# andrewdalpino/UltraZoom

Hardware: AMD Instinct MI355X
Metric: upscaled MPix/sec, MewZoom-4X 1080p bf16 batched inference (higher is better)
Workload: dtype bf16; 1 GPU; MewZoom-4X 96ch/40L bf16, 16 x 1080x1920 -> 4320x7680 per GPU; global_batch=16, parallelism=batch-sharded x1, images_in_flight=0

## Files before the change

### include/mewzoom_hip.h

```cpp
#ifndef MEWZOOM_HIP_H
#define MEWZOOM_HIP_H

#include <stddef.h>
#include <stdint.h>

#ifdef __cplusplus
extern "C" {
#endif

typedef struct mz_handle mz_handle;

typedef enum mz_dtype {
    MZ_F32 = 0,
    MZ_BF16 = 1,
    MZ_F16 = 2
} mz_dtype;

typedef enum mz_status {
    MZ_OK = 0,
    MZ_ERR_INVALID_ARGUMENT = -1,
    MZ_ERR_UNKNOWN_WEIGHT = -2,
    MZ_ERR_SHAPE_MISMATCH = -3,
    MZ_ERR_MISSING_WEIGHTS = -4,
    MZ_ERR_WORKSPACE_TOO_SMALL = -5,
// ... 100 lines not shown
const char* mz_version(void);
double mz_flops_per_image(const mz_handle* h, int H, int W);
int mz_profile_enable(mz_handle* h, int on);
int mz_profile_dump(mz_handle* h, const char* path);
int mz_profile_read(mz_handle* h, double* conv_ms, double* conv_flops, double* conv_launches,
                    double* other_ms, double* conv_bytes);

int mz_debug_read(unsigned long long* host_dst);

const char* mz_debug_last_kernel(void);

int mz_debug_tile_list(int B, int tiles_y, int tiles_x, int ntiles, int gm, int gn, int blk4, int th, int tw, unsigned int* out, int cap);

const char* mz_debug_select(int dtype, int op, int cin, int cout, int B, int H, int W, int cus);

typedef struct mz_debug_step {
    int32_t kind, op, cin, cout, B, H, W, Hout, Wout, fused;
    int64_t off[3];
    uint64_t bytes[3];
    const char* kernel;
} mz_debug_step;

int mz_debug_schedule(const mz_handle* h, int B, int H, int W, int want_qa, int cus, mz_debug_step* out, int cap);

long long mz_debug_pack(int dtype, int op, int cin, int cout, int layout, long long* out, long long cap);

int mz_debug_store_hazard(int follower, int form, int wait_states, int dword, int iters, int blocks, unsigned int* counts_out);

#ifdef __cplusplus
}
// ... 3 lines not shown
```

### ultrazoom_amd/csrc/mz_conv3r.h

```cpp
#pragma once
#include "mz_device.h"
#include "mz_diag.h"
#include "mz_relay.h"

namespace mz {
namespace r3 {

constexpr int TH = 8;
template <int GEO> struct Geo {
    static_assert(GEO == 0 || GEO == 1, "8 x 48 or 8 x 40");
    static constexpr int TW = GEO == 0 ? 48 : 40;
    static constexpr int NPF = GEO == 0 ? 6 : 5;
    static constexpr int ROWW = TW + 2;
    static constexpr int NPIX = 10 * ROWW;
    static constexpr int DIV_MAGIC = GEO == 0 ? 1311 : 1561;
    static constexpr int X0 = 3, X1 = NPF - 3;
    static constexpr bool straddle(int pf) { return GEO == 1 && pf == 2; }
    static constexpr int dy(int pf) { return GEO == 0 ? pf / 3 : (pf >= 3 ? 1 : 0); }
    static constexpr int dx(int pf) { return GEO == 0 ? 16 * (pf % 3) : (pf < 2 ? 16 * pf : (pf == 2 ? 0 : 8 + 16 * (pf - 3))); }
};
constexpr int PLANE_ENT = 512;
constexpr int A_PLANE = PLANE_ENT * 16;
constexpr int A_SLOT = 4 * A_PLANE;
constexpr int NT = 3, NF = 6, BN = 96;
constexpr int NG = 9 * NT;
constexpr int B_BASE = 2 * A_SLOT;
constexpr int CHUNK_PIECES = 2 * NG;
constexpr int MIX_PIECES = 4 * NT * NT;

template <int NSEG> struct Seg {
    static_assert(NSEG == 2 || NSEG == 3, "two or three weight segments per chunk");
    static constexpr int start(int s) { return NSEG == 2 ? (s <= 0 ? 0 : (s == 1 ? (NG + 1) / 2 : NG)) : (NG / 3) * s; }
    static constexpr int of(int G) { return NSEG == 2 ? (G < start(1) ? 0 : 1) : G / (NG / 3); }
    static constexpr int pieces(int s) { return 2 * (start(s + 1) - start(s)); }
    static constexpr int SLOT = pieces(0) * 1024;
    static constexpr int MIX_BASE = B_BASE + 3 * SLOT;
    static constexpr int lds_bytes(bool fuse) { return fuse ? MIX_BASE + MIX_PIECES * 1024 : B_BASE + 3 * SLOT; }
};

template <int GEO, int TAP, int PF> constexpr int a_off() {
    using GG = Geo<GEO>;
    constexpr int DY = TAP / 3, DX = TAP % 3;
    return ((DY + GG::dy(PF)) * GG::ROWW + DX + GG::dx(PF)) * 16;
}

template <int NPF> struct Frag {
    u32x4 x[2][NPF];
    u32x4 w[3][2];
};

template <int N> __device__ __forceinline__ void wait_w(u32x4& w0, u32x4& w1) {
    asm volatile("s_waitcnt lgkmcnt(%2)" : "+v"(w0), "+v"(w1) : "n"(N) : "memory");
// ... 95 lines not shown
        gate_wait<(more ? NT : 0)>(wa);
        __builtin_amdgcn_sched_barrier(0);
#pragma unroll
        for (int i = 0; i < NT; ++i) {
            if constexpr (ks == 0) mma16_first<TT>(beta[part * NT + i], wa[i], xf[0]);
            else if constexpr (ks < NT) mma16<TT>(beta[part * NT + i], wa[i], xf[ks]);
            else mma16<TT>(beta[part * NT + i], wa[i], zf[ks - NT]);
        }
        __builtin_amdgcn_sched_barrier(0);
        gate_halves<TT, H + 1>(beta, xf, zf, wb, wa, addr);
    }
}

}

template <class TT, int NSEG, int EPI, bool SILU, int GEO = 0, bool RAG = false>
__global__ __launch_bounds__(512) void conv3r_kernel(const ConvArgs a) {
    using namespace r3;
    using namespace relay;
    using S = Seg<NSEG>;
    using GG = Geo<GEO>;
    constexpr int NPF = GG::NPF, TW = GG::TW, ROWW = GG::ROWW, NPIX = GG::NPIX;
    constexpr int NE = NPF * NT;
    constexpr bool FUSE = EPI == EPI_FUSEDMIX;
    static_assert(!FUSE || GEO == 0, "the fused variant is built for the 8 x 48 tile");
    constexpr int B_SLOT = S::SLOT;
    static_assert(!FUSE || NSEG == 3, "the gate weights need the LDS that three weight segments leave free");
    static_assert(!RAG || (NSEG == 3 && EPI == EPI_STORE && GEO == 0), "the ragged two-chunk variant: three steps per chunk, plain stores, 8 x 48 tiles");
    extern __shared__ __attribute__((aligned(16))) char smem[];
    const int w = __builtin_amdgcn_readfirstlane((int)threadIdx.x >> 6);
    const int team = w >> 2, wq = w & 3;
    const int nchunks = a.nchunks16;
    const uint32_t lds_base = (uint32_t)(uintptr_t)(__attribute__((address_space(3))) char*)smem;

    const int xcd = blockIdx.x & 7, pos = blockIdx.x >> 3, step = gridDim.x >> 3;
    const int q = a.grid >> 3, rem = a.grid & 7;
    const int cnt = q + (xcd < rem ? 1 : 0);
    const int base = xcd < rem ? xcd * (q + 1) : rem * (q + 1) + (xcd - rem) * q;
    if (pos >= cnt) return;
    typedef uint32_t TabE __attribute__((ext_vector_type(2)));
    typedef const __attribute__((address_space(4))) TabE* TabPtr;
    const TabPtr tab = (TabPtr)(uintptr_t)a.tile_tab + base;
    struct TileE { uint32_t yx, bn; };
// ... 217 lines not shown
    auto entry_whole = [&](auto e_tag) __attribute__((always_inline)) {
        if constexpr (decltype(e_tag)::value < NE) {
            u32x4 o;
            entry_words(e_tag, o);
            epi_store(e_tag, o);
        }
    };

    auto prime = [&](int wslot, int aslot) __attribute__((always_inline)) {
        const int lane_ = lane_now();
        const int g = lane_ >> 4, c = lane_ & 15;
        Bases pb;
        pb.a_cur = pb.a_nxt = lds_base + aslot * A_SLOT + g * A_PLANE + ((2 * wq) * ROWW + c) * 16;
        pb.a2_cur = pb.a2_nxt = pb.a_cur + (uint32_t)((c >= 8 ? ROWW - 8 : 32) * 16);
        pb.b_cur = pb.b_nxt = 0;
        const uint32_t bb = lds_base + B_BASE + wslot * B_SLOT + lane_ * 16;
        f.x[0][0] = read_x<GEO, 0, 0>(pb, false);
        f.x[0][1] = read_x<GEO, 0, 1>(pb, false);
        f.x[0][2] = read_x<GEO, 0, 2>(pb, false);
        f.x[0][3] = read_x<GEO, 0, 3>(pb, false);
        f.x[0][4] = read_x<GEO, 0, 4>(pb, false);
        if constexpr (NPF > 5) f.x[0][NPF - 1] = read_x<GEO, 0, NPF - 1>(pb, false);
        f.w[0][0] = lds_read128<0 * 1024>(bb);
        f.w[0][1] = lds_read128<1 * 1024>(bb);
        f.w[1][0] = lds_read128<2 * 1024>(bb);
        f.w[1][1] = lds_read128<3 * 1024>(bb);
        wait_wx<0>(f.w[0][0], f.w[0][1], f.x[0]);
        wait_w<0>(f.w[1][0], f.w[1][1]);
    };

    const char* wA = nullptr;
    const char* wB = nullptr;
    bool okB = false;
    auto loader_step = [&](auto wk_tag, auto es_tag, auto en_tag, auto sg_tag, auto last_tag, int k) __attribute__((always_inline)) {
        constexpr int WK = decltype(wk_tag)::value;
        constexpr int ES = decltype(es_tag)::value, EN = WK == 0 ? 0 : decltype(en_tag)::value, sg = decltype(sg_tag)::value;
        constexpr bool last = decltype(last_tag)::value != 0;
        [[maybe_unused]] constexpr int rs_c = 1 + (EN > 0 ? 2 : 0) + (sg == 0 ? 0 : 1);
        static_assert(EN <= 3, "three output registers");
        constexpr int VM_AFTER0 = WK == 1 ? EN : (WK == 2 ? (ES + 1 < NPF ? NF : 0) : (WK == 4 ? EN * NT : 0));
        constexpr int VM_AFTER = VM_AFTER0 + (NSEG == 3 && sg == 0 ? 8 : 0);
        RS_BEGIN();
        if constexpr (WK == 2 && ES == 0) fuse_x(ic<0>{});
        if constexpr (WK == 3) x_landed(ic<ES>{});
        constexpr bool HALO_LATE = NSEG == 3;
        auto halo_image = [&]() __attribute__((always_inline)) {
            const __amdgpu_buffer_rsrc_t h_rsrc = halo_rsrc(last ? 0 : k + 1);
            uint32_t h_off = (uint32_t)(us ^ 1) * (uint32_t)A_SLOT;
// ... 4 lines not shown
            halo_piece(ic<3>{}, h_rsrc, h_dst, rag); halo_piece(ic<4>{}, h_rsrc, h_dst, rag); halo_piece(ic<5>{}, h_rsrc, h_dst, rag);
            halo_piece(ic<6>{}, h_rsrc, h_dst, rag); halo_piece(ic<7>{}, h_rsrc, h_dst, rag);
        };
        if constexpr (sg == 0 && !HALO_LATE) {
            if (!last || okB) halo_image();
        }
        {
            constexpr bool same = sg + 2 < NSEG;
            constexpr int qs = same ? sg + 2 : sg + 2 - NSEG;
            const char* wsrc;
            bool w_ok = true;
            if constexpr (same) wsrc = wA + (size_t)k * chunk_bytes;
            else if constexpr (!last) wsrc = wA + (size_t)(k + 1) * chunk_bytes;
            else { wsrc = wB; w_ok = okB; }
            wsrc += (size_t)(2 * S::start(qs)) * 1024;
            const int w_pieces = w_ok ? wseg_count(S::pieces(qs)) : 0;
            char* const w_dst = smem + B_BASE + (hs >= 1 ? hs - 1 : 2) * B_SLOT;
            const uint32_t lo = (uint32_t)lane_now() * 16u;
            wseg_piece(ic<0>{}, wsrc, w_pieces, w_dst, lo); wseg_piece(ic<1>{}, wsrc, w_pieces, w_dst, lo); wseg_piece(ic<2>{}, wsrc, w_pieces, w_dst, lo);
            wseg_piece(ic<3>{}, wsrc, w_pieces, w_dst, lo); wseg_piece(ic<4>{}, wsrc, w_pieces, w_dst, lo);
            if constexpr (WP > 5) wseg_piece(ic<5>{}, wsrc, w_pieces, w_dst, lo);
            if constexpr (WP > 6) wseg_piece(ic<6>{}, wsrc, w_pieces, w_dst, lo);
            static_assert(WP <= 7, "seven weight pieces per wave and step");
        }
        if constexpr (sg == 0 && HALO_LATE) halo_image();
        __builtin_amdgcn_sched_barrier(0);
        asm volatile("" ::: "memory");
        RS_LAP(4 * rs_c);
        if constexpr (WK == 1) {
            u32x4 o0, o1, o2;
            if constexpr (EN > 0) entry_words(ic<ES>{}, o0);
            if constexpr (EN > 1) entry_words(ic<ES + 1>{}, o1);
// ... 48 lines not shown
    auto fuse_chunk = [&](auto p0_tag, auto g_tag, auto last_tag, int k) __attribute__((always_inline)) {
        static_assert(!FUSE || NSEG == 3, "the fused variant runs three steps per chunk");
        loader_step(ic<2>{}, p0_tag, g_tag, ic<0>{}, last_tag, k);
        loader_step(ic<3>{}, p0_tag, g_tag, ic<1>{}, last_tag, k);
        loader_step(ic<4>{}, p0_tag, g_tag, ic<NSEG - 1>{}, last_tag, k);
    };
    auto plain_chunks = [&](int k0) __attribute__((always_inline)) {
        for (int k = k0; k + 1 < nchunks; ++k) loader_chunk(ic<0>{}, ic<0>{}, ic<0>{}, ic<0>{}, k);
        loader_chunk(ic<0>{}, ic<0>{}, ic<0>{}, ic<1>{}, nchunks - 1);
    };
    auto loader_phase = [&](auto epi_tag) __attribute__((always_inline)) {
        constexpr bool DO_EPI = decltype(epi_tag)::value != 0;
        wA = wsrc_of(tile_nt(eA));
        okB = a_pos + step < cnt;
        wB = wsrc_of(tile_nt(okB ? eB : eA));
        const TileE eA2 = tile_at(a_pos + 2 * step), eB2 = tile_at(a_pos + 3 * step);
        if constexpr (DO_EPI) {
            RS_BEGIN();
            set_load_tile(eA);
            epi_setup();
            RS_FENCE();
            RS_LAP(27);
            if constexpr (RAG) {
                loader_chunk(ic<0>{}, ic<3>{}, ic<6>{}, ic<0>{}, 0);
                loader_chunk(ic<9>{}, ic<3>{}, ic<6>{}, ic<1>{}, 1);
            } else if constexpr (FUSE) {
                fuse_chunk(ic<0>{}, ic<1>{}, ic<0>{}, 0);
                fuse_chunk(ic<1>{}, ic<1>{}, ic<0>{}, 1);
                fuse_chunk(ic<2>{}, ic<1>{}, ic<0>{}, 2);
                fuse_chunk(ic<3>{}, ic<1>{}, ic<0>{}, 3);
// ... 33 lines not shown
        eD = eB; eA = eA2; eB = eB2;
        asm volatile("" ::"s"(eA.yx), "s"(eA.bn), "s"(eB.yx), "s"(eB.bn));
    };

    auto compute_phase = [&]() __attribute__((always_inline)) {
        const int lane_ = lane_now();
        const int g = lane_ >> 4, c = lane_ & 15;
        const uint32_t a_lane = lds_base + g * A_PLANE + ((2 * wq) * ROWW + c) * 16;
        Bases bs;
        bs.a_cur = a_lane + us * A_SLOT;
        bs.a_nxt = a_lane + (us ^ 1) * A_SLOT;
        const uint32_t a_str = (uint32_t)((c >= 8 ? ROWW - 8 : 32) * 16);
        bs.a2_cur = bs.a_cur + a_str;
        bs.a2_nxt = bs.a_nxt + a_str;
        const uint32_t bl = lds_base + B_BASE + lane_ * 16;
        uint32_t b0 = bl + hs * B_SLOT, b1 = bl + next3(hs) * B_SLOT, b2 = bl + next3(next3(hs)) * B_SLOT;
        bs.b_cur = b0;
        bs.b_nxt = b1;
        auto step_tail = [&]() __attribute__((always_inline)) {
            __builtin_amdgcn_s_barrier();
            const uint32_t u_ = b0; b0 = b1; b1 = b2; b2 = u_;
            bs.b_cur = b0; bs.b_nxt = b1;
        };
        auto chunk = [&](auto xp_tag, bool first) __attribute__((always_inline)) {
            constexpr int XP = decltype(xp_tag)::value;
            groups<TT, NSEG, GEO, S::start(0), S::start(1), XP>(acc, f, bs, first);
            step_tail();
            groups<TT, NSEG, GEO, S::start(1), S::start(2), XP>(acc, f, bs, false);
            step_tail();
            if constexpr (NSEG == 3) {
                groups<TT, NSEG, GEO, S::start(2), S::start(3), XP>(acc, f, bs, false);
                step_tail();
            }
            const uint32_t v_ = bs.a_cur; bs.a_cur = bs.a_nxt; bs.a_nxt = v_;
            if constexpr (GEO == 1) { const uint32_t v2_ = bs.a2_cur; bs.a2_cur = bs.a2_nxt; bs.a2_nxt = v2_; }
        };
        RS_BEGIN();
        int kc = 0;
        for (;;) {
            chunk(ic<0>{}, !FUSE && kc == 0);
            if (++kc >= nchunks) break;
            chunk(ic<1>{}, false);
            if (++kc >= nchunks) break;
        }
        asm volatile("s_waitcnt lgkmcnt(0)"
                     : "+v"(f.x[0][0]), "+v"(f.x[0][1]), "+v"(f.x[0][2]), "+v"(f.x[0][3]), "+v"(f.x[0][4]), "+v"(f.x[0][NPF - 1]),
                       "+v"(f.x[1][0]), "+v"(f.x[1][1]), "+v"(f.x[1][2]), "+v"(f.x[1][3]), "+v"(f.x[1][4]), "+v"(f.x[1][NPF - 1])
// ... 26 lines not shown
        }
    };

    if (team == 1) {
        eA = tile_at(a_pos);
        eB = tile_at(a_pos + step);
        eD = eA;
        wA = wsrc_of(tile_nt(eA));
        set_load_tile(eA);
        {
            const __amdgpu_buffer_rsrc_t r0 = halo_rsrc(0);
            halo_piece(ic<0>{}, r0, smem); halo_piece(ic<1>{}, r0, smem); halo_piece(ic<2>{}, r0, smem); halo_piece(ic<3>{}, r0, smem);
            halo_piece(ic<4>{}, r0, smem); halo_piece(ic<5>{}, r0, smem); halo_piece(ic<6>{}, r0, smem); halo_piece(ic<7>{}, r0, smem);
            const char* s1 = wA + (size_t)(2 * S::start(1)) * 1024;
            const uint32_t lo = (uint32_t)lane_now() * 16u;
            char* d0 = smem + B_BASE;
            char* d1 = smem + B_BASE + B_SLOT;
            wseg_piece(ic<0>{}, wA, wseg_count(S::pieces(0)), d0, lo); wseg_piece(ic<1>{}, wA, wseg_count(S::pieces(0)), d0, lo); wseg_piece(ic<2>{}, wA, wseg_count(S::pieces(0)), d0, lo);
            wseg_piece(ic<3>{}, wA, wseg_count(S::pieces(0)), d0, lo); wseg_piece(ic<4>{}, wA, wseg_count(S::pieces(0)), d0, lo); wseg_piece(ic<5>{}, wA, wseg_count(S::pieces(0)), d0, lo);
            wseg_piece(ic<6>{}, wA, wseg_count(S::pieces(0)), d0, lo);
            wseg_piece(ic<0>{}, s1, wseg_count(S::pieces(1)), d1, lo); wseg_piece(ic<1>{}, s1, wseg_count(S::pieces(1)), d1, lo); wseg_piece(ic<2>{}, s1, wseg_count(S::pieces(1)), d1, lo);
            wseg_piece(ic<3>{}, s1, wseg_count(S::pieces(1)), d1, lo); wseg_piece(ic<4>{}, s1, wseg_count(S::pieces(1)), d1, lo); wseg_piece(ic<5>{}, s1, wseg_count(S::pieces(1)), d1, lo);
            wseg_piece(ic<6>{}, s1, wseg_count(S::pieces(1)), d1, lo);
        }
        if constexpr (FUSE) {
            const int lane_ = lane_now();
            const char* msrc = (const char*)a.wmix16 + (uint32_t)lane_ * 16u;
#pragma unroll
            for (int i = 0; i < MIX_PIECES / 4; ++i) glds16(msrc + (size_t)(wq + 4 * i) * 1024, smem + S::MIX_BASE + (wq + 4 * i) * 1024);
        }
        wait_vmcnt<0>();
        __builtin_amdgcn_s_barrier();
// ... 31 lines not shown
```

### ultrazoom_amd/csrc/mz_conv3r.hip

```cpp
#include "mz_conv3r.h"

#ifndef MZ_R_NSEG
#define MZ_R_NSEG 3
#endif

namespace mz {

template <class TT, int NSEG, int EPI, bool SILU = false, int GEO = 0, bool RAG = false> static hipError_t r_launch(const ConvArgs& a, hipStream_t s) {
    constexpr size_t lds = r3::Seg<NSEG>::lds_bytes(EPI == EPI_FUSEDMIX);
    return launch_lds<conv3r_kernel<TT, NSEG, EPI, SILU, GEO, RAG>>(a.persist, 512, lds, a, s);
}
template <class TT> static hipError_t r_epi(const ConvArgs& a, hipStream_t s) {
    if (a.ragged_planes) {
        if (a.nchunks16 != 2 || a.ragged_planes < 1 || a.ragged_planes > 3 || a.epi != EPI_STORE || !a.silu || a.geo != 0) return hipErrorInvalidValue;
        return r_launch<TT, 3, EPI_STORE, true, 0, true>(a, s);
    }
    if (a.nchunks16 < 3) return hipErrorInvalidValue;
    if (a.geo == 1) {
        switch (a.epi) {
            case EPI_STORE: return a.silu ? r_launch<TT, MZ_R_NSEG, EPI_STORE, true, 1>(a, s) : r_launch<TT, MZ_R_NSEG, EPI_STORE, false, 1>(a, s);
            case EPI_D2S: return r_launch<TT, MZ_R_NSEG, EPI_D2S, false, 1>(a, s);
            default: return hipErrorInvalidValue;
        }
    }
    switch (a.epi) {
        case EPI_STORE: return a.silu ? r_launch<TT, MZ_R_NSEG, EPI_STORE, true>(a, s) : r_launch<TT, MZ_R_NSEG, EPI_STORE, false>(a, s);
        case EPI_D2S: return r_launch<TT, MZ_R_NSEG, EPI_D2S>(a, s);
        case EPI_FUSEDMIX: return a.wmix16 ? r_launch<TT, 3, EPI_FUSEDMIX>(a, s) : hipErrorInvalidValue;
        default: return hipErrorInvalidValue;
    }
}

hipError_t launch_conv3r(int dtype, const ConvArgs& a, hipStream_t s) {
    if (a.persist <= 0 || (a.persist & 7) || a.nchunks16 < 2 || a.geo < 0 || a.geo > 1) return hipErrorInvalidValue;
    switch (dtype) {
        case DT_BF16: return r_epi<TBF16>(a, s);
        case DT_F16: return r_epi<TF16>(a, s);
        default: return hipErrorInvalidValue;
    }
}

}
```

### ultrazoom_amd/csrc/mz_debug.cpp

```cpp
#include <cstdarg>
#include <cstdio>

#include "mz_host.h"
#include "mz_pack.h"

using namespace mz;

static thread_local char g_err[512] = "";
thread_local const char* mz::g_last_kernel = "";
int mz::fail(int code, const char* fmt, ...) {
    va_list ap;
    va_start(ap, fmt);
    vsnprintf(g_err, sizeof(g_err), fmt, ap);
    va_end(ap);
    return code;
}
extern "C" const char* mz_last_error(void) { return g_err; }
extern "C" const char* mz_debug_last_kernel(void) { return g_last_kernel; }

int mz::device_cus() {
    static int known[kMaxDevices];
    int n = 0, dev = 0;
    if (hipGetDeviceCount(&n) != hipSuccess || n <= 0) return fail(MZ_ERR_NO_DEVICE, "no HIP device visible");
    if (hipGetDevice(&dev) != hipSuccess || dev < 0 || dev >= kMaxDevices) return fail(MZ_ERR_NO_DEVICE, "bad current device");
    if (!known[dev]) {
        int c = 0;
        if (hipDeviceGetAttribute(&c, hipDeviceAttributeMultiprocessorCount, dev) != hipSuccess) c = 0;
        known[dev] = c / 8 * 8 + 1;
    }
    return known[dev] - 1;
}

extern "C" int mz_debug_read(unsigned long long* host_dst) {
// ... 2 lines not shown
    return hipMemcpy(host_dst, b, 16 * 64 * 8 * sizeof(unsigned long long), hipMemcpyDeviceToHost) == hipSuccess ? 0 : -6;
}

extern "C" int mz_debug_tile_list(int B, int tiles_y, int tiles_x, int ntiles, int gm, int gn, int blk4, int th, int tw, unsigned int* out, int cap) {
    if (B < 1 || tiles_x < 1 || tiles_y < 1 || ntiles < 1 || gm < 1 || gn < 1 || th < 1 || tw < 1 || !out || cap < 0) return MZ_ERR_INVALID_ARGUMENT;
    const int mtiles = B * tiles_x * tiles_y;
    std::vector<uint32_t> t;
    tile_list(group_walk(tiles_x, tiles_y, mtiles, ntiles, std::min(gm, mtiles), std::min(gn, ntiles), blk4 ? 1 : 0), th, tw, t);
    const int n = (int)(t.size() / 2);
    for (int i = 0; i < n && i < cap; ++i) { out[2 * i] = t[2 * i]; out[2 * i + 1] = t[2 * i + 1]; }
    return n;
}

template <class T> static T refused(T nothing, const Refusal& r) { fail(r); return nothing; }

extern "C" const char* mz_debug_select(int dtype, int op, int cin, int cout, int B, int H, int W, int cus) {
    const char* const none = nullptr;
    if ((dtype != MZ_F32 && dtype != MZ_BF16 && dtype != MZ_F16) || cin < 1 || cout < 1 || B < 1 || H < 1 || W < 1 || cus < 0)
        return refused(none, refuse(MZ_ERR_INVALID_ARGUMENT, "bad arguments"));
    if (op == 5 && dtype != DT_BF16 && dtype != DT_F16)
        return refused(none, refuse(MZ_ERR_INVALID_ARGUMENT, "the FiLM epilogue is implemented for bf16 / fp16"));
    if (op == 8) return refused(none, refuse(MZ_ERR_INVALID_ARGUMENT, "bad op %d", op));
    const Knobs k = read_knobs();
    BlockPlan b;
    Refusal why;
    const LayerPlan* c = plan_debug_layer(b, dtype, op, cin, cout, &why);
    if (!c) return refused(none, why);
    if (op == 7) return kernel_name(choose_mix(k, dtype, *c, B, H, W, cus));
    Conv3Call call;
    switch (op) {
        case 0: call = conv1_call(*c, nullptr, nullptr, B, H, W); break;
        case 2: call = d2s_call(*c, nullptr, nullptr, B, H, W, 2 * H, 2 * W); break;
        case 3: call = head_call(*c, nullptr, nullptr, B, H, W); break;
        case 5: call = film_call(*c, nullptr, nullptr, B, H, W, 0); break;
        case 6: call = conv2_call(k, b, nullptr, nullptr, B, H, W); break;
        default: call = plain_call(*c, nullptr, nullptr, B, H, W); break;
    }
    const KernelChoice ch = choose_conv3(k, dtype, call, cus);
    return ch.ok ? kernel_name(ch) : refused(none, refuse(MZ_ERR_INVALID_ARGUMENT, "%s", ch.why));
}

extern "C" long long mz_debug_pack(int dtype, int op, int cin, int cout, int layout, long long* out, long long cap) {
    if ((dtype != MZ_F32 && dtype != MZ_BF16 && dtype != MZ_F16) || cin < 1 || cout < 1 || layout < 0 || layout >= PK_COUNT || cap < 0 ||
        (cap > 0 && !out))
        return refused(-1LL, refuse(MZ_ERR_INVALID_ARGUMENT, "bad arguments"));
    BlockPlan b;
    Refusal why;
    const LayerPlan* c = plan_debug_layer(b, dtype, op, cin, cout, &why);
    if (!c) return refused(-1LL, why);
    if (!c->has(layout)) return refused(-1LL, refuse(MZ_ERR_INVALID_ARGUMENT, "the layer has no packing %d", layout));
    const PackArgs p = pack_args(*c, layout, dtype, nullptr, nullptr);
    const long long n = (long long)(packed_bytes(p.taps, p.frags, p.ntiles, p.nchunks) / dtype_size(dtype));
    for (long long i = 0; i < n && i < cap; ++i) out[i] = dtype == DT_F32 ? pack_source<4>(p, i) : pack_source<2>(p, i);
    return n;
// ... 41 lines not shown
```

### ultrazoom_amd/csrc/mz_err.h

```cpp
#pragma once
#include <hip/hip_runtime.h>

#include "mz_view_check.h"

namespace mz {

extern thread_local const char* g_last_kernel;

__attribute__((format(printf, 2, 3))) int fail(int code, const char* fmt, ...);
inline int fail(const Refusal& r) { return fail(r.code, "%s", r.msg); }
inline int hip_rc(hipError_t e, const char* what) { return e == hipSuccess ? MZ_OK : fail(MZ_ERR_HIP, "%s: %s", what, hipGetErrorString(e)); }
#define HIPCHK(expr) do { if (int rc_ = hip_rc((expr), #expr " failed")) return rc_; } while (0)

int device_cus();

}
```

### ultrazoom_amd/csrc/mz_kernels.h

```cpp
#pragma once
#include <hip/hip_runtime.h>
#include <stddef.h>
#include <stdint.h>

namespace mz {

enum DType : int { DT_F32 = 0, DT_BF16 = 1, DT_F16 = 2 };

inline int dtype_size(int dt) { return dt == DT_F32 ? 4 : 2; }
inline int chunk_channels(int dt) { return dt == DT_F32 ? 8 : 16; }
inline int pad16(int c) { return (c + 15) / 16 * 16; }

enum ConvMode : int { MODE_CONV3 = 0, MODE_GEMM1 = 1, MODE_C3W16 = 2, MODE_C3W8 = 3 };
enum SrcKind : int { SRC_PLAIN = 0, SRC_CONCAT = 1, SRC_CRUSH = 2, SRC_MIXF = 3  };
enum Epilogue : int {
    EPI_STORE = 0,
    EPI_D2S = 1,
    EPI_MIX = 2,
    EPI_FINAL = 3,
    EPI_FUSEDMIX = 4,
};

struct ConvArgs {
    const void* in0;
// ... 31 lines not shown
    float inv_mix_scale;
    int R;
    int Hi, Wi;
    int clamp;
    int io_u8;
    int persist;
    int s16;
    const void* wpk16;
    int nchunks16;
    const void* tile_tab;
    int ragged_planes;
    int geo;
    const void* wmix16;
    const float* film_gamma;
    const float* film_beta;
    int use_glds;
    unsigned long long* dbg;
    int view;
    long long vin[4], vout[4];
    int win_y0, win_x0, win_h, win_w;
};

struct ImageViews {
    long long in[4], out[4];
    int y0, x0, h, w;
};

inline int choose_nt(int n_padded) {
    const int order[4] = {3, 2, 4, 1};
    int best = 1, best_n = 1 << 30;
    for (int i = 0; i < 4; ++i) {
// ... 72 lines not shown
```

### ultrazoom_amd/csrc/mz_plan.h

```cpp
#pragma once
#include <stdlib.h>

#include <algorithm>
#include <vector>

#include "mz_geo.h"

namespace mz {

struct Knobs {
    bool wide = true;
    bool fuse = true;
    bool s16 = true;
    bool fuse16 = true;
    bool mix16b = true;
    int persist = -1;
    int kpad_pct = 12;
    int blk4 = 1;
    int r = 1;
    int r2 = 1;
    int t = 1;
};
inline Knobs read_knobs() {
    Knobs k;
    k.wide = getenv("MZ_NO_WIDE") == nullptr;
    k.fuse = getenv("MZ_NO_FUSE") == nullptr;
    k.s16 = getenv("MZ_NO_S16") == nullptr;
    k.fuse16 = getenv("MZ_NO_FUSE16") == nullptr;
    k.mix16b = getenv("MZ_NO_MIX16B") == nullptr;
    k.r = getenv("MZ_NO_R") == nullptr;
    k.t = getenv("MZ_NO_T") == nullptr;
    k.r2 = getenv("MZ_NO_R2") == nullptr;
    k.blk4 = getenv("MZ_NO_BLK4") == nullptr;
    if (const char* e = getenv("MZ_KPAD_PCT")) k.kpad_pct = atoi(e);
    if (getenv("MZ_NO_PERSIST") != nullptr) k.persist = 0;
    else if (const char* e = getenv("MZ_PERSIST_WGS")) { const int n = atoi(e) / 8 * 8; k.persist = n > 0 ? n : 0; }
    return k;
}

struct LayerPlan {
    int cout = 0, cin = 0, kh = 0, kw = 0;
    int mode = MODE_CONV3, taps = 9, nt = 1, ntiles = 1, nchunks = 1, nchunks_real = 1;
    int out_map = OUT_PLAIN, cq = 0, cq_p = 0;
    int in_map = SRC_PLAIN, c0 = 0, cp0 = 0, c1 = 0;
    int n_logical_padded = 0;
    int nchunks32 = 0;
    unsigned layouts = 0;
    bool has(int layout) const { return layouts >> layout & 1u; }
};

struct PackShape { int frags, ntiles, nchunks; };
// ... 197 lines not shown
```

### ultrazoom_amd/csrc/mz_runner.h

```cpp
#pragma once
#include <cmath>
#include <cstring>
#include <map>
#include <utility>

#include "mz_err.h"
#include "mz_select.h"

namespace mz {

struct DevBuf {
    void* p = nullptr;
    DevBuf() = default;
    DevBuf(DevBuf&& o) noexcept : p(o.p) { o.p = nullptr; }
    ~DevBuf() {
        if (p) (void)hipFree(p);
    }
    hipError_t alloc(size_t bytes) { return p ? hipSuccess : hipMalloc(&p, bytes); }
};

struct ConvW : LayerPlan {
    DevBuf packed[PK_COUNT];
};
using BlockW = Block<ConvW>;
// ... 117 lines not shown

    hipError_t launch_kernel(const KernelChoice& ch, const ConvArgs& a, int nt) {
        switch (ch.kernel) {
            case K_CONV256: return launch_conv256(dtype, ch.mode, nt, a, s);
            case K_CONV3W: return launch_conv3w(dtype, ch.mode, nt, a, s);
            case K_CONV3P: return launch_conv3p(dtype, ch.mode, nt, a, s);
            case K_CONV3S: return launch_conv3s(dtype, ch.mode, nt, a, s);
            case K_CONV3R: return launch_conv3r(dtype, a, s);
            case K_CONV3T: return launch_conv3t(dtype, a, s);
            case K_MIX16: return launch_mix16(dtype, a, s);
            case K_MIX16B: return launch_mix16b(dtype, a, s, ch.persist);
        }
        return hipErrorInvalidValue;
    }
    void launch(const KernelChoice& ch, const ConvArgs& a, int nt, ProfRec* r, const char* what = nullptr) {
        if (!what) what = g_last_kernel = kernel_name(ch);
        check(launch_kernel(ch, a, nt), what);
        if (r) (void)hipEventRecord(r->b, s);
    }

    void conv3(const Conv3Call& k) {
        if (rc) return;
        const KernelChoice ch = choose_conv3(knobs, dtype, k, cus);
        if (!ch.ok) { rc = fail(MZ_ERR_INVALID_ARGUMENT, "%s", ch.why); return; }
        const ConvW& c = weights(k.c);
        const int B = k.B, H = k.H, W = k.W;
        const double sz = dtype_size(dtype);
        const double px = (double)B * H * W;
        const int tiles_x = (W + ch.tw - 1) / ch.tw, tiles_y = (H + ch.th - 1) / ch.th;
        const Walk w = pick_order(tiles_x, tiles_y, B * tiles_x * tiles_y, c.ntiles, (double)pack_bytes(c, PK_MAIN), px * c.cp0 * sz, knobs);
        ConvArgs a;
// ... 10 lines not shown
        }
        const bool fused = ch.fused;
        if (fused) {
            a.in1 = k.xin;
            a.p1 = pad16(c.cout) * dtype_size(dtype) / 16;
            a.wmix = weights(k.mixf).packed[PK_MAIN].p;
            a.mix_pieces = k.mixf->nchunks * k.mixf->nt;
            const int slot = ch.mode == MODE_C3W16 ? stage_bytes<MODE_C3W16>(c.nt) : stage_bytes<MODE_C3W8>(c.nt);
            const int ncx = a.p1 / 2;
            a.x_via_lds = (a.mix_pieces * 1024 + 8 * ncx * 1024 <= 2 * slot) ? 1 : 0;
            a.mix_scale = 1.0f / (1.0f + std::exp(-k.alpha));
            a.inv_mix_scale = inv_sigmoid(k.alpha);
        }
        a.geo = ch.geo;
        a.ragged_planes = ch.ragged_planes;
        if (ch.layout != PK_MAIN) {
            a.wpk16 = c.packed[ch.layout].p;
            a.nchunks16 = pack_shape(c, ch.layout).nchunks;
            if (fused) a.wmix16 = weights(k.mixf).packed[ch.gate].p;
        }
        if (ch.tile_list) tile_table(a, w, ch.th, ch.tw, ch.persist);
        if (rc) return;
        a.persist = std::min((a.grid + 7) / 8 * 8, ch.persist);
        a.film_gamma = k.gamma; a.film_beta = k.beta;
        const double flops = 2.0 * px * 9.0 * c.cin * c.cout + (fused ? 2.0 * px * 2.0 * c.cout * c.cout : 0.0);
        const double bytes = px * (c.cin + c.cout) * sz + 9.0 * c.cin * c.cout * sz + (fused ? px * c.cout * sz : 0.0);
        launch(ch, a, c.nt, prof_begin(0, a, c, flops, bytes));
    }

    void mix(const ConvW& c, float alpha, const void* x, const void* z, void* out, int B, int H, int W) {
// ... 43 lines not shown
```

### ultrazoom_amd/csrc/mz_select.h

```cpp
#pragma once
#include <math.h>

#include <vector>

#include "mz_plan.h"
#include "mz_view_check.h"

namespace mz {

struct Walk {
    int tiles_x = 0, tiles_y = 0;
    int mtiles = 0, ntiles = 0;
    int gm = 1, gn = 1, groups_m = 0, grid = 0;
    int blk4 = 0;
    float inv_gsz = 1.f, inv_groups_m = 1.f, inv_gn = 1.f, inv_tpi = 1.f, inv_tiles_x = 1.f, inv_bsz = 1.f;
};

inline Walk group_walk(int tiles_x, int tiles_y, int mtiles, int ntiles, int gm, int gn, int blk4) {
    Walk w;
    w.tiles_x = tiles_x; w.tiles_y = tiles_y; w.mtiles = mtiles; w.ntiles = ntiles;
    w.gm = gm; w.gn = gn; w.blk4 = blk4;
    w.groups_m = (mtiles + gm - 1) / gm;
    w.grid = (int)((long long)w.groups_m * ((ntiles + gn - 1) / gn) * gm * gn);
    w.inv_gsz = 1.0f / (float)(gm * gn);
// ... 50 lines not shown
        t.push_back((uint32_t)(tyi * th) | (uint32_t)(txi * tw) << 16);
        t.push_back((uint32_t)b | (uint32_t)nt << 16);
    }
}

struct KernelChoice {
    bool ok = false;
    const char* why = nullptr;
    int kernel = K_CONV256;
    int mode = MODE_GEMM1;
    bool fused = false;
    bool mix = false;
    int th = 0, tw = 0;
    int geo = 0;
    int ragged_planes = 0;
    int layout = PK_MAIN;
    int gate = PK_MAIN;
    bool tile_list = false;
    int persist = 0;
};

inline const char* kernel_name(const KernelChoice& ch) {
    if (!ch.ok) return nullptr;
    switch (ch.kernel) {
        case K_CONV256: return ch.mix ? "conv_kernel_mix" : "conv_kernel";
        case K_CONV3W: return ch.fused ? (ch.persist > 0 ? "conv3p" : "conv3w_fused") : "conv3w";
        case K_CONV3P: return "conv3p";
        case K_CONV3S: return ch.fused ? "conv3s_fused" : "conv3s";
        case K_CONV3R: return ch.fused ? "conv3r_fused" : ch.ragged_planes ? "conv3r_ragged" : ch.geo ? "conv3r_8x40" : "conv3r";
        case K_CONV3T: return ch.fused ? "conv3t_fused" : "conv3t";
        case K_MIX16: return "mix16";
        case K_MIX16B: return "mix16b";
    }
    return nullptr;
}

inline int persistent_workgroups(const Knobs& k, int cus) { return k.persist >= 0 ? k.persist : cus; }

inline bool offsets_fit(double planes, double pixels) { return planes * pixels * 16.0 < 4294967296.0; }

struct Conv3Call {
    const LayerPlan* c = nullptr;
    const LayerPlan* mixf = nullptr;
    int epi = EPI_STORE, silu = 0;
    bool film = false;
    int B = 0, H = 0, W = 0, Hout = 0, Wout = 0;
    const void* in = nullptr;
    void* out = nullptr;
    const void* xin = nullptr;
// ... 81 lines not shown
    }

    if (k.r && k.fuse16 && epi == EPI_FUSEDMIX && s16 && c.nt == 3 && c.ntiles == 1 && c.has(PK_CONV16) && mixf && mixf->has(PK_GATE16R) &&
        mixf->nchunks32 == c.nt && c.nchunks32 >= 6 && p0 % 4 == 0 && k_fits && halo_fits && offsets_fit(12, px))
        return listed(K_CONV3R, 8, 48, PK_CONV16, PK_GATE16R);

    if (k.r && s16 && !call.film && c.nt == 3 && c.has(PK_CONV16) && (epi == EPI_STORE || epi == EPI_D2S) && k_fits && halo_fits &&
        c.nchunks32 >= 3 && p0 % 4 == 0 &&
        (epi == EPI_D2S ? offsets_fit(c.cq_p * dtype_size(dtype) / 16, (double)call.Hout * call.Wout) : offsets_fit(12, px))) {
        const long long rows8 = (long long)((H + 7) / 8 * 8);
        const long long pad48 = rows8 * ((W + 47) / 48 * 48), pad40 = rows8 * ((W + 39) / 40 * 40);
        const long long pads = (long long)((H + th - 1) / th) * th * ((W + tw - 1) / tw) * tw;
        const int geo = pad40 < pad48 ? 1 : 0;
        if ((geo ? pad40 : pad48) <= pads) {
            ch.geo = geo;
            return listed(K_CONV3R, 8, geo ? 40 : 48, PK_CONV16, PK_MAIN);
        }
    }

    ch.th = th; ch.tw = tw;
    ch.fused = fused;
    const bool fuse16 = fused && mixf && mixf->has(PK_GATE16) && k.fuse16 &&
                        mixf->nchunks32 == c.nt;
    if (mode != MODE_CONV3 && (epi == EPI_STORE || epi == EPI_D2S || fuse16) && wgs > 0) {
        const int tiles_x = (W + tw - 1) / tw, tiles_y = (H + th - 1) / th;
        const Walk g = pick_order(tiles_x, tiles_y, B * tiles_x * tiles_y, c.ntiles, (double)pack_bytes(c, PK_MAIN),
                                  (double)B * H * W * c.cp0 * (double)dtype_size(dtype), k);
        if (s16 && c.has(PK_CONV16) && k_fits && halo_fits) {
            ch.layout = PK_CONV16;
            ch.gate = fused ? PK_GATE16 : PK_MAIN;
// ... 56 lines not shown
```

Measured before the change: 698.0 MPix/s.

## Keep one weight segment per chunk resident in LDS for conv3r kernels

Adds a WRES variant of the conv3r kernel. For layers with exactly three 32-channel weight chunks, one segment of every chunk is kept resident in LDS, and only the other two segments stream through a two-slot ring. The resident segment is reloaded only when a persistent workgroup moves to a tile with a different output-channel tile. The aim is to cut repeated global-to-LDS weight traffic, at the cost of a larger LDS footprint per workgroup (five slots instead of three), which may reduce occupancy. It is enabled by default, with an env switch to turn it off, plus debug hooks that report the chosen variant.

```diff
diff --git a/include/mewzoom_hip.h b/include/mewzoom_hip.h
--- a/include/mewzoom_hip.h
+++ b/include/mewzoom_hip.h
@@ -138,6 +138,9 @@
 
 const char* mz_debug_select(int dtype, int op, int cin, int cout, int B, int H, int W, int cus);
 
+const char* mz_debug_last_variant(void);
+const char* mz_debug_select_variant(int dtype, int op, int cin, int cout, int B, int H, int W, int cus);
+
 typedef struct mz_debug_step {
     int32_t kind, op, cin, cout, B, H, W, Hout, Wout, fused;
     int64_t off[3];
diff --git a/ultrazoom_amd/csrc/mz_conv3r.h b/ultrazoom_amd/csrc/mz_conv3r.h
--- a/ultrazoom_amd/csrc/mz_conv3r.h
+++ b/ultrazoom_amd/csrc/mz_conv3r.h
@@ -2,6 +2,10 @@
 #include "mz_device.h"
 #include "mz_diag.h"
 #include "mz_relay.h"
+
+#ifndef MZ_R_RES_SEG
+#define MZ_R_RES_SEG 0
+#endif
 
 namespace mz {
 namespace r3 {
@@ -36,6 +40,11 @@
     static constexpr int SLOT = pieces(0) * 1024;
     static constexpr int MIX_BASE = B_BASE + 3 * SLOT;
     static constexpr int lds_bytes(bool fuse) { return fuse ? MIX_BASE + MIX_PIECES * 1024 : B_BASE + 3 * SLOT; }
+    static constexpr int RES_SEG = MZ_R_RES_SEG, RING_SLOT = 3;
+    static_assert(RES_SEG >= 0 && RES_SEG < 3, "the resident segment of a chunk");
+    static constexpr int ring_slot(int seg) { return RING_SLOT + (seg - RES_SEG - 1 + 3) % 3; }
+    static constexpr int wres_slot(int seg, int k) { return seg == RES_SEG ? k : ring_slot(seg); }
+    static constexpr int lds_bytes_wres() { return B_BASE + 5 * SLOT; }
 };
 
 template <int GEO, int TAP, int PF> constexpr int a_off() {
@@ -161,7 +170,7 @@
 
 }
 
-template <class TT, int NSEG, int EPI, bool SILU, int GEO = 0, bool RAG = false>
+template <class TT, int NSEG, int EPI, bool SILU, int GEO = 0, bool RAG = false, bool WRES = false>
 __global__ __launch_bounds__(512) void conv3r_kernel(const ConvArgs a) {
     using namespace r3;
     using namespace relay;
@@ -174,6 +183,7 @@
     constexpr int B_SLOT = S::SLOT;
     static_assert(!FUSE || NSEG == 3, "the gate weights need the LDS that three weight segments leave free");
     static_assert(!RAG || (NSEG == 3 && EPI == EPI_STORE && GEO == 0), "the ragged two-chunk variant: three steps per chunk, plain stores, 8 x 48 tiles");
+    static_assert(!WRES || (NSEG == 3 && !FUSE && !RAG), "resident weight segments: three steps per chunk, unfused (the fused variant's gate weights fill the LDS), whole chunks");
     extern __shared__ __attribute__((aligned(16))) char smem[];
     const int w = __builtin_amdgcn_readfirstlane((int)threadIdx.x >> 6);
     const int team = w >> 2, wq = w & 3;
@@ -421,7 +431,7 @@
         pb.a_cur = pb.a_nxt = lds_base + aslot * A_SLOT + g * A_PLANE + ((2 * wq) * ROWW + c) * 16;
         pb.a2_cur = pb.a2_nxt = pb.a_cur + (uint32_t)((c >= 8 ? ROWW - 8 : 32) * 16);
         pb.b_cur = pb.b_nxt = 0;
-        const uint32_t bb = lds_base + B_BASE + wslot * B_SLOT + lane_ * 16;
+        const uint32_t bb = lds_base + B_BASE + (WRES ? S::wres_slot(0, 0) : wslot) * B_SLOT + lane_ * 16;
         f.x[0][0] = read_x<GEO, 0, 0>(pb, false);
         f.x[0][1] = read_x<GEO, 0, 1>(pb, false);
         f.x[0][2] = read_x<GEO, 0, 2>(pb, false);
@@ -439,6 +449,7 @@
     const char* wA = nullptr;
     const char* wB = nullptr;
     bool okB = false;
+    [[maybe_unused]] bool relA = false, relB = false;
     auto loader_step = [&](auto wk_tag, auto es_tag, auto en_tag, auto sg_tag, auto last_tag, int k) __attribute__((always_inline)) {
         constexpr int WK = decltype(wk_tag)::value;
         constexpr int ES = decltype(es_tag)::value, EN = WK == 0 ? 0 : decltype(en_tag)::value, sg = decltype(sg_tag)::value;
@@ -473,8 +484,19 @@
             else if constexpr (!last) wsrc = wA + (size_t)(k + 1) * chunk_bytes;
             else { wsrc = wB; w_ok = okB; }
             wsrc += (size_t)(2 * S::start(qs)) * 1024;
+            char* w_dst;
+            if constexpr (WRES) {
+                if constexpr (qs == S::RES_SEG) {
+                    if constexpr (same) { w_ok = relA; w_dst = smem + B_BASE + k * B_SLOT; }
+                    else if constexpr (!last) { w_ok = relA; w_dst = smem + B_BASE + (k + 1) * B_SLOT; }
+                    else { w_ok = okB && relB; w_dst = smem + B_BASE; }
+                } else {
+                    w_dst = smem + B_BASE + S::ring_slot(qs) * B_SLOT;
+                }
+            } else {
+                w_dst = smem + B_BASE + (hs >= 1 ? hs - 1 : 2) * B_SLOT;
+            }
             const int w_pieces = w_ok ? wseg_count(S::pieces(qs)) : 0;
-            char* const w_dst = smem + B_BASE + (hs >= 1 ? hs - 1 : 2) * B_SLOT;
             const uint32_t lo = (uint32_t)lane_now() * 16u;
             wseg_piece(ic<0>{}, wsrc, w_pieces, w_dst, lo); wseg_piece(ic<1>{}, wsrc, w_pieces, w_dst, lo); wseg_piece(ic<2>{}, wsrc, w_pieces, w_dst, lo);
             wseg_piece(ic<3>{}, wsrc, w_pieces, w_dst, lo); wseg_piece(ic<4>{}, wsrc, w_pieces, w_dst, lo);
@@ -553,6 +575,10 @@
         wA = wsrc_of(tile_nt(eA));
         okB = a_pos + step < cnt;
         wB = wsrc_of(tile_nt(okB ? eB : eA));
+        if constexpr (WRES) {
+            relA = tile_nt(eA) != tile_nt(eD);
+            relB = tile_nt(eB) != tile_nt(eA);
+        }
         const TileE eA2 = tile_at(a_pos + 2 * step), eB2 = tile_at(a_pos + 3 * step);
         if constexpr (DO_EPI) {
             RS_BEGIN();
@@ -616,23 +642,34 @@
         bs.a2_cur = bs.a_cur + a_str;
         bs.a2_nxt = bs.a_nxt + a_str;
         const uint32_t bl = lds_base + B_BASE + lane_ * 16;
-        uint32_t b0 = bl + hs * B_SLOT, b1 = bl + next3(hs) * B_SLOT, b2 = bl + next3(next3(hs)) * B_SLOT;
-        bs.b_cur = b0;
-        bs.b_nxt = b1;
-        auto step_tail = [&]() __attribute__((always_inline)) {
+        uint32_t b0 = WRES ? bl : bl + hs * B_SLOT, b1 = WRES ? bl + S::RING_SLOT * B_SLOT : bl + next3(hs) * B_SLOT,
+                 b2 = WRES ? bl + (S::RING_SLOT + 1) * B_SLOT : bl + next3(next3(hs)) * B_SLOT;
+        [[maybe_unused]] auto wres_addr = [&](int seg) __attribute__((always_inline)) {
+            return seg == S::RES_SEG ? b0 : (S::ring_slot(seg) == S::RING_SLOT ? b1 : b2);
+        };
+        bs.b_cur = WRES ? wres_addr(0) : b0;
+        bs.b_nxt = WRES ? wres_addr(1) : b1;
+        auto step_tail = [&]([[maybe_unused]] auto sg_tag) __attribute__((always_inline)) {
             __builtin_amdgcn_s_barrier();
-            const uint32_t u_ = b0; b0 = b1; b1 = b2; b2 = u_;
-            bs.b_cur = b0; bs.b_nxt = b1;
+            if constexpr (WRES) {
+                constexpr int sg = decltype(sg_tag)::value;
+                if constexpr (sg == S::RES_SEG) b0 += B_SLOT;
+                bs.b_cur = wres_addr((sg + 1) % 3);
+                bs.b_nxt = wres_addr((sg + 2) % 3);
+            } else {
+                const uint32_t u_ = b0; b0 = b1; b1 = b2; b2 = u_;
+                bs.b_cur = b0; bs.b_nxt = b1;
+            }
         };
         auto chunk = [&](auto xp_tag, bool first) __attribute__((always_inline)) {
             constexpr int XP = decltype(xp_tag)::value;
             groups<TT, NSEG, GEO, S::start(0), S::start(1), XP>(acc, f, bs, first);
-            step_tail();
+            step_tail(ic<0>{});
             groups<TT, NSEG, GEO, S::start(1), S::start(2), XP>(acc, f, bs, false);
-            step_tail();
+            step_tail(ic<1>{});
             if constexpr (NSEG == 3) {
                 groups<TT, NSEG, GEO, S::start(2), S::start(3), XP>(acc, f, bs, false);
-                step_tail();
+                step_tail(ic<2>{});
             }
             const uint32_t v_ = bs.a_cur; bs.a_cur = bs.a_nxt; bs.a_nxt = v_;
             if constexpr (GEO == 1) { const uint32_t v2_ = bs.a2_cur; bs.a2_cur = bs.a2_nxt; bs.a2_nxt = v2_; }
@@ -689,8 +726,17 @@
             halo_piece(ic<4>{}, r0, smem); halo_piece(ic<5>{}, r0, smem); halo_piece(ic<6>{}, r0, smem); halo_piece(ic<7>{}, r0, smem);
             const char* s1 = wA + (size_t)(2 * S::start(1)) * 1024;
             const uint32_t lo = (uint32_t)lane_now() * 16u;
-            char* d0 = smem + B_BASE;
-            char* d1 = smem + B_BASE + B_SLOT;
+            char* d0 = smem + B_BASE + (WRES ? S::wres_slot(0, 0) : 0) * B_SLOT;
+            char* d1 = smem + B_BASE + (WRES ? S::wres_slot(1, 0) : 1) * B_SLOT;
+            if constexpr (WRES) {
+#pragma unroll
+                for (int c = S::RES_SEG < 2 ? 1 : 0; c < 3; ++c) {
+                    const char* sc = wA + (size_t)c * chunk_bytes + (size_t)(2 * S::start(S::RES_SEG)) * 1024;
+                    char* dc = smem + B_BASE + c * B_SLOT;
+                    wseg_piece(ic<0>{}, sc, wseg_count(S::pieces(0)), dc, lo); wseg_piece(ic<1>{}, sc, wseg_count(S::pieces(0)), dc, lo); wseg_piece(ic<2>{}, sc, wseg_count(S::pieces(0)), dc, lo);
+                    wseg_piece(ic<3>{}, sc, wseg_count(S::pieces(0)), dc, lo); wseg_piece(ic<4>{}, sc, wseg_count(S::pieces(0)), dc, lo);
+                }
+            }
             wseg_piece(ic<0>{}, wA, wseg_count(S::pieces(0)), d0, lo); wseg_piece(ic<1>{}, wA, wseg_count(S::pieces(0)), d0, lo); wseg_piece(ic<2>{}, wA, wseg_count(S::pieces(0)), d0, lo);
             wseg_piece(ic<3>{}, wA, wseg_count(S::pieces(0)), d0, lo); wseg_piece(ic<4>{}, wA, wseg_count(S::pieces(0)), d0, lo); wseg_piece(ic<5>{}, wA, wseg_count(S::pieces(0)), d0, lo);
             wseg_piece(ic<6>{}, wA, wseg_count(S::pieces(0)), d0, lo);
diff --git a/ultrazoom_amd/csrc/mz_conv3r.hip b/ultrazoom_amd/csrc/mz_conv3r.hip
--- a/ultrazoom_amd/csrc/mz_conv3r.hip
+++ b/ultrazoom_amd/csrc/mz_conv3r.hip
@@ -6,27 +6,34 @@
 
 namespace mz {
 
-template <class TT, int NSEG, int EPI, bool SILU = false, int GEO = 0, bool RAG = false> static hipError_t r_launch(const ConvArgs& a, hipStream_t s) {
-    constexpr size_t lds = r3::Seg<NSEG>::lds_bytes(EPI == EPI_FUSEDMIX);
-    return launch_lds<conv3r_kernel<TT, NSEG, EPI, SILU, GEO, RAG>>(a.persist, 512, lds, a, s);
+template <class TT, int NSEG, int EPI, bool SILU = false, int GEO = 0, bool RAG = false, bool WRES = false> static hipError_t r_launch(const ConvArgs& a, hipStream_t s) {
+    constexpr size_t lds = WRES ? r3::Seg<NSEG>::lds_bytes_wres() : r3::Seg<NSEG>::lds_bytes(EPI == EPI_FUSEDMIX);
+    return launch_lds<conv3r_kernel<TT, NSEG, EPI, SILU, GEO, RAG, WRES>>(a.persist, 512, lds, a, s);
+}
+template <class TT, int EPI, bool SILU, int GEO> static hipError_t r_plain(const ConvArgs& a, hipStream_t s) {
+    if (a.wres) {
+        if (a.nchunks16 != 3) return hipErrorInvalidValue;
+        return r_launch<TT, 3, EPI, SILU, GEO, false, true>(a, s);
+    }
+    return r_launch<TT, MZ_R_NSEG, EPI, SILU, GEO>(a, s);
 }
 template <class TT> static hipError_t r_epi(const ConvArgs& a, hipStream_t s) {
     if (a.ragged_planes) {
-        if (a.nchunks16 != 2 || a.ragged_planes < 1 || a.ragged_planes > 3 || a.epi != EPI_STORE || !a.silu || a.geo != 0) return hipErrorInvalidValue;
+        if (a.wres || a.nchunks16 != 2 || a.ragged_planes < 1 || a.ragged_planes > 3 || a.epi != EPI_STORE || !a.silu || a.geo != 0) return hipErrorInvalidValue;
         return r_launch<TT, 3, EPI_STORE, true, 0, true>(a, s);
     }
     if (a.nchunks16 < 3) return hipErrorInvalidValue;
     if (a.geo == 1) {
         switch (a.epi) {
-            case EPI_STORE: return a.silu ? r_launch<TT, MZ_R_NSEG, EPI_STORE, true, 1>(a, s) : r_launch<TT, MZ_R_NSEG, EPI_STORE, false, 1>(a, s);
-            case EPI_D2S: return r_launch<TT, MZ_R_NSEG, EPI_D2S, false, 1>(a, s);
+            case EPI_STORE: return a.silu ? r_plain<TT, EPI_STORE, true, 1>(a, s) : r_plain<TT, EPI_STORE, false, 1>(a, s);
+            case EPI_D2S: return r_plain<TT, EPI_D2S, false, 1>(a, s);
             default: return hipErrorInvalidValue;
         }
     }
     switch (a.epi) {
-        case EPI_STORE: return a.silu ? r_launch<TT, MZ_R_NSEG, EPI_STORE, true>(a, s) : r_launch<TT, MZ_R_NSEG, EPI_STORE, false>(a, s);
-        case EPI_D2S: return r_launch<TT, MZ_R_NSEG, EPI_D2S>(a, s);
-        case EPI_FUSEDMIX: return a.wmix16 ? r_launch<TT, 3, EPI_FUSEDMIX>(a, s) : hipErrorInvalidValue;
+        case EPI_STORE: return a.silu ? r_plain<TT, EPI_STORE, true, 0>(a, s) : r_plain<TT, EPI_STORE, false, 0>(a, s);
+        case EPI_D2S: return r_plain<TT, EPI_D2S, false, 0>(a, s);
+        case EPI_FUSEDMIX: return a.wmix16 && !a.wres ? r_launch<TT, 3, EPI_FUSEDMIX>(a, s) : hipErrorInvalidValue;
         default: return hipErrorInvalidValue;
     }
 }
diff --git a/ultrazoom_amd/csrc/mz_debug.cpp b/ultrazoom_amd/csrc/mz_debug.cpp
--- a/ultrazoom_amd/csrc/mz_debug.cpp
+++ b/ultrazoom_amd/csrc/mz_debug.cpp
@@ -16,7 +16,9 @@
     return code;
 }
 extern "C" const char* mz_last_error(void) { return g_err; }
+thread_local const char* mz::g_last_variant = "";
 extern "C" const char* mz_debug_last_kernel(void) { return g_last_kernel; }
+extern "C" const char* mz_debug_last_variant(void) { return g_last_variant; }
 
 int mz::device_cus() {
     static int known[kMaxDevices];
@@ -49,7 +51,7 @@
 
 template <class T> static T refused(T nothing, const Refusal& r) { fail(r); return nothing; }
 
-extern "C" const char* mz_debug_select(int dtype, int op, int cin, int cout, int B, int H, int W, int cus) {
+static const char* debug_select(int dtype, int op, int cin, int cout, int B, int H, int W, int cus, bool variant) {
     const char* const none = nullptr;
     if ((dtype != MZ_F32 && dtype != MZ_BF16 && dtype != MZ_F16) || cin < 1 || cout < 1 || B < 1 || H < 1 || W < 1 || cus < 0)
         return refused(none, refuse(MZ_ERR_INVALID_ARGUMENT, "bad arguments"));
@@ -61,7 +63,10 @@
     Refusal why;
     const LayerPlan* c = plan_debug_layer(b, dtype, op, cin, cout, &why);
     if (!c) return refused(none, why);
-    if (op == 7) return kernel_name(choose_mix(k, dtype, *c, B, H, W, cus));
+    if (op == 7) {
+        const KernelChoice mx = choose_mix(k, dtype, *c, B, H, W, cus);
+        return variant ? kernel_variant(mx) : kernel_name(mx);
+    }
     Conv3Call call;
     switch (op) {
         case 0: call = conv1_call(*c, nullptr, nullptr, B, H, W); break;
@@ -72,7 +77,14 @@
         default: call = plain_call(*c, nullptr, nullptr, B, H, W); break;
     }
     const KernelChoice ch = choose_conv3(k, dtype, call, cus);
-    return ch.ok ? kernel_name(ch) : refused(none, refuse(MZ_ERR_INVALID_ARGUMENT, "%s", ch.why));
+    if (!ch.ok) return refused(none, refuse(MZ_ERR_INVALID_ARGUMENT, "%s", ch.why));
+    return variant ? kernel_variant(ch) : kernel_name(ch);
+}
+extern "C" const char* mz_debug_select(int dtype, int op, int cin, int cout, int B, int H, int W, int cus) {
+    return debug_select(dtype, op, cin, cout, B, H, W, cus, false);
+}
+extern "C" const char* mz_debug_select_variant(int dtype, int op, int cin, int cout, int B, int H, int W, int cus) {
+    return debug_select(dtype, op, cin, cout, B, H, W, cus, true);
 }
 
 extern "C" long long mz_debug_pack(int dtype, int op, int cin, int cout, int layout, long long* out, long long cap) {
diff --git a/ultrazoom_amd/csrc/mz_err.h b/ultrazoom_amd/csrc/mz_err.h
--- a/ultrazoom_amd/csrc/mz_err.h
+++ b/ultrazoom_amd/csrc/mz_err.h
@@ -6,6 +6,7 @@
 namespace mz {
 
 extern thread_local const char* g_last_kernel;
+extern thread_local const char* g_last_variant;
 
 __attribute__((format(printf, 2, 3))) int fail(int code, const char* fmt, ...);
 inline int fail(const Refusal& r) { return fail(r.code, "%s", r.msg); }
diff --git a/ultrazoom_amd/csrc/mz_kernels.h b/ultrazoom_amd/csrc/mz_kernels.h
--- a/ultrazoom_amd/csrc/mz_kernels.h
+++ b/ultrazoom_amd/csrc/mz_kernels.h
@@ -69,7 +69,7 @@
     const void* wmix16;
     const float* film_gamma;
     const float* film_beta;
-    int use_glds;
+    int wres;
     unsigned long long* dbg;
     int view;
     long long vin[4], vout[4];
diff --git a/ultrazoom_amd/csrc/mz_plan.h b/ultrazoom_amd/csrc/mz_plan.h
--- a/ultrazoom_amd/csrc/mz_plan.h
+++ b/ultrazoom_amd/csrc/mz_plan.h
@@ -20,7 +20,11 @@
     int r = 1;
     int r2 = 1;
     int t = 1;
-};
+    int wres = 1;
+};
+inline void read_variant_switches(Knobs& k) {
+    k.wres = getenv("MZ_NO_WRES") == nullptr;
+}
 inline Knobs read_knobs() {
     Knobs k;
     k.wide = getenv("MZ_NO_WIDE") == nullptr;
@@ -35,6 +39,7 @@
     if (const char* e = getenv("MZ_KPAD_PCT")) k.kpad_pct = atoi(e);
     if (getenv("MZ_NO_PERSIST") != nullptr) k.persist = 0;
     else if (const char* e = getenv("MZ_PERSIST_WGS")) { const int n = atoi(e) / 8 * 8; k.persist = n > 0 ? n : 0; }
+    read_variant_switches(k);
     return k;
 }
 
diff --git a/ultrazoom_amd/csrc/mz_runner.h b/ultrazoom_amd/csrc/mz_runner.h
--- a/ultrazoom_amd/csrc/mz_runner.h
+++ b/ultrazoom_amd/csrc/mz_runner.h
@@ -155,7 +155,10 @@
         return hipErrorInvalidValue;
     }
     void launch(const KernelChoice& ch, const ConvArgs& a, int nt, ProfRec* r, const char* what = nullptr) {
-        if (!what) what = g_last_kernel = kernel_name(ch);
+        if (!what) {
+            what = g_last_kernel = kernel_name(ch);
+            g_last_variant = kernel_variant(ch);
+        }
         check(launch_kernel(ch, a, nt), what);
         if (r) (void)hipEventRecord(r->b, s);
     }
@@ -196,6 +199,7 @@
         }
         a.geo = ch.geo;
         a.ragged_planes = ch.ragged_planes;
+        a.wres = ch.wres ? 1 : 0;
         if (ch.layout != PK_MAIN) {
             a.wpk16 = c.packed[ch.layout].p;
             a.nchunks16 = pack_shape(c, ch.layout).nchunks;
diff --git a/ultrazoom_amd/csrc/mz_select.h b/ultrazoom_amd/csrc/mz_select.h
--- a/ultrazoom_amd/csrc/mz_select.h
+++ b/ultrazoom_amd/csrc/mz_select.h
@@ -88,6 +88,7 @@
     int th = 0, tw = 0;
     int geo = 0;
     int ragged_planes = 0;
+    bool wres = false;
     int layout = PK_MAIN;
     int gate = PK_MAIN;
     bool tile_list = false;
@@ -107,6 +108,10 @@
         case K_MIX16B: return "mix16b";
     }
     return nullptr;
+}
+
+inline const char* kernel_variant(const KernelChoice& ch) {
+    return ch.ok && ch.kernel == K_CONV3R && ch.wres ? "wres" : "";
 }
 
 inline int persistent_workgroups(const Knobs& k, int cus) { return k.persist >= 0 ? k.persist : cus; }
@@ -218,6 +223,7 @@
         const int geo = pad40 < pad48 ? 1 : 0;
         if ((geo ? pad40 : pad48) <= pads) {
             ch.geo = geo;
+            ch.wres = k.wres && c.nchunks32 == 3;
             return listed(K_CONV3R, 8, geo ? 40 : 48, PK_CONV16, PK_MAIN);
         }
     }
```

Result: no change. 699.8 MPix/s, median of 6 (+0.3%).
